# andrepxx/go-dsp-guitar

Hardware: AMD Instinct MI355X
Metric: Msamples/s through full chain incl. 64k-tap cab IR, 512ch@192kHz; %HBM roofline (higher is better)
Workload: dtype f64

## Files before the change

go-dsp-guitar_amd/csrc/api_ctx.cpp:

```cpp
#include "ctx.h"

static const int g_param_count[GDG_UNIT_COUNT] = { 6, 3, 3, 5, 4, 3, 7, 3, 7, 6, 4, 4, 2, 2, 3, 3, 1, 3, 1, 1, 1 };
static const int32_t g_param_default[GDG_UNIT_COUNT][GDG_MAX_PARAMS] = {
    { 100, 0, 0, 440, 100, 0 }, { -20, -40, 50 }, { 0, 300, 3000 }, { 1, -40, -10, 300, 6000 },
    { 1, -40, -10, 100 }, { 1, 30, -20 }, { 1, -20, -20, -20, -20, -20, -20 }, { 0, 0, 0 },
    { 1, 50, 0, 0, 100, 0, 0 }, { 0, 0, 100, 0, 1, 0 }, { 0, 0, 0, 0 }, { 0, -2, -5, -5 },
    { 100, 30 }, { 100, 10 }, { 100, 10, 45 }, { 100, 50, -10 }, { 100 }, { 200, -5, -5 }, { 50 }, { 14 }, { 0 },
};


const char *gdg_version(void) { return "gdg 0.1 gfx950 hip"; }

int gdg_device_count(void) {
    int n = 0;
    if (hipGetDeviceCount(&n) != hipSuccess) return 0;
    return n;
}


static bool parse_cpulist(const char *text, std::vector<int> &cpus) {
    cpus.clear();
    const char *p = text;
    while (*p && *p != '\n') {
        char *end = nullptr;
// ... 76 lines not shown
hipError_t pinned_alloc(gdg_ctx *ctx, void **p, size_t bytes) {
    const std::vector<int> *unused;
    const int node = numa_target(ctx, &unused);
    const bool bind = node >= 0 && node < 1024;
    if (bind) {
        unsigned long mask[16] = { 0 };
        mask[node / (8 * sizeof(unsigned long))] |= 1ul << (node % (8 * sizeof(unsigned long)));
        int old_mode = 0;
        unsigned long old_mask[16] = { 0 };
        const bool saved = syscall(SYS_get_mempolicy, &old_mode, old_mask, 1024ul + 1, nullptr, 0ul) == 0;
        const bool policy = saved && syscall(SYS_set_mempolicy, 1 , mask, 1024ul + 1) == 0;
        hipError_t e = hipHostMalloc(p, bytes, policy ? hipHostMallocNumaUser : hipHostMallocDefault);
        if (policy && syscall(SYS_set_mempolicy, old_mode, old_mode == 0 ? nullptr : old_mask, old_mode == 0 ? 0ul : 1024ul + 1) != 0)
            syscall(SYS_set_mempolicy, 0 , nullptr, 0ul);
        if (e == hipSuccess) return e;
        (void)hipGetLastError();
    }
    return hipHostMalloc(p, bytes, hipHostMallocDefault);
}

struct OptionDef {
    const char *key, *env;
    long long lo, hi;
    int knob;
    int gdg_ctx::*field;
    bool gdg_ctx::*flag;
    bool replans;
};
static const OptionDef g_options[] = {
    { "fir_fused", "GDG_FIR_FUSED", -1, 1, -1, &gdg_ctx::fir_fused, nullptr, true },
    { "fir_split_max_channels", "GDG_FIR_SPLIT_MAX", 0, 1 << 20, -1, &gdg_ctx::fir_split_max, nullptr, true },
    { "fir_split_max_channels_one_amp", "GDG_FIR_SPLIT_MAX_ONE_AMP", 0, 1 << 20, -1, &gdg_ctx::fir_split_max_single, nullptr, true },
    { "fir_chain_adjacent_amps", "GDG_FIR_CHAIN", 0, 1, -1, nullptr, &gdg_ctx::fir_chain, true },
    { "fir_premac", "GDG_FIR_PREMAC", 0, 1, -1, &gdg_ctx::fir_premac, nullptr, true },
    { "fir_premac_min_partitions", "GDG_FIR_PREMAC_MIN", 1, 1 << 24, -1, &gdg_ctx::fir_premac_min, nullptr, true },
    { "fir_premac_min_partitions_two_amps", "GDG_FIR_PREMAC_MIN_TWO", 1, 1 << 24, -1, &gdg_ctx::fir_premac_min_two, nullptr, true },
    { "stat_premac_launches_used", "GDG_STAT_PREMAC_USED", 0, 0x7fffffff, -1, &gdg_ctx::stat_premac_used, nullptr, false },
    { "stat_batch_device_kib", "GDG_STAT_BATCH_DEVICE_KIB", 0, 0x7fffffff, -1, &gdg_ctx::stat_batch_dev_kib, nullptr, false },
    { "stat_batch_upload_bytes", "GDG_STAT_BATCH_UPLOAD_BYTES", 0, 0x7fffffff, -1, &gdg_ctx::stat_batch_up_bytes, nullptr, false },
    { "stat_batch_resampled_samples", "GDG_STAT_BATCH_RESAMPLED", 0, 0x7fffffff, -1, &gdg_ctx::stat_batch_resampled, nullptr, false },
    { "fir_ahead_frames", "GDG_FIR_AHEAD", 0, 4, -1, &gdg_ctx::fir_ahead_frames, nullptr, true },
    { "fir_ahead_min_channels", "GDG_FIR_AHEAD_MIN", 1, 1 << 20, -1, &gdg_ctx::fir_ahead_min, nullptr, true },
    { "stat_fir_ahead_sums_used", "GDG_STAT_FIR_AHEAD_USED", 0, 0x7fffffff, -1, &gdg_ctx::stat_fir_ahead_used, nullptr, false },
    { "fir_premac_lds_bytes", "GDG_FIR_PREMAC_LDS", -1, 65536, -1, &gdg_ctx::fir_premac_lds, nullptr, true },
    { "share_ir_spectra", "GDG_SHARE_IR_SPECTRA", 0, 1, -1, nullptr, &gdg_ctx::share_spectra, false },
    { "fft_half_lds_mask", "GDG_FFT_HALF_LDS", 0, 63, GDG_KNOB_FFT_HALF_LDS, nullptr, nullptr, false },
    { "fir_forward_per_channel", "GDG_FWD_PER_CHANNEL", 0, 1, GDG_KNOB_FWD_PER_CHANNEL, nullptr, nullptr, false },
    { "fir_forward_wave_local", "GDG_WAVE_FFT", 0, 3, GDG_KNOB_WAVE_FFT, nullptr, nullptr, false },
    { "fir_mac_variant", "GDG_MAC_VARIANT", 0, 15, GDG_KNOB_MAC_VARIANT, nullptr, nullptr, false },
    { "seg_two_per_cu", "GDG_SEG_FAST", 0, 1, -1, nullptr, &gdg_ctx::seg_fast, true },
    { "seg_two_per_cu_min_channels", "GDG_SEG_FAST_MIN", 0, 1 << 20, -1, &gdg_ctx::seg_fast_min, nullptr, true },
    { "seg_wave_max_channels", "GDG_SEG_WAVE_MAX", 0, 1 << 20, -1, &gdg_ctx::seg_wave_max, nullptr, true },
    { "seg_wave_release_max_channels", "GDG_SEG_WAVE_RELEASE_MAX", 0, 1 << 20, -1, &gdg_ctx::seg_wave_release_max, nullptr, true },
    { "seg_tile_max_channels", "GDG_SEG_TILE_MAX", 0, 1 << 20, -1, &gdg_ctx::seg_tile_max, nullptr, true },
    { "seg_os_tiles_max_channels", "GDG_SEG_OS_TILES_MAX", 0, 1 << 20, -1, &gdg_ctx::seg_os_tiles_max, nullptr, true },
    { "seg_os_tiles_prefix", "GDG_SEG_OS_PREFIX", 0, 1, -1, nullptr, &gdg_ctx::seg_os_prefix, true },
    { "seg_reverb_ahead_max_channels", "GDG_SEG_REVERB_AHEAD_MAX", 0, 1 << 20, -1, &gdg_ctx::seg_reverb_ahead_max, nullptr, true },
    { "wave_spin_limit_ms", "GDG_WAVE_SPIN_LIMIT_MS", 1, 600000, -1, &gdg_ctx::wave_spin_ms, nullptr, false },
    { "debug_stall_unit", "GDG_DEBUG_STALL_UNIT", -1, 1 << 30, -1, &gdg_ctx::debug_stall_unit, nullptr, false },
    { "plan_patch", "GDG_PLAN_PATCH", 0, 1, -1, nullptr, &gdg_ctx::plan_patch, false },
    { "scan_tables_max", "GDG_SCAN_TABLES_MAX", 1, 1 << 20, -1, &gdg_ctx::scan_tables_max, nullptr, false },
    { "pcie_groups", "GDG_PCIE_GROUPS", 0, 16, -1, &gdg_ctx::pcie_groups_forced, nullptr, false },
    { "device_groups_default", "GDG_DEVICE_GROUPS", 0, 16, -1, &gdg_ctx::device_groups_env, nullptr, false },
    { "copy_threads", "GDG_COPY_THREADS", 1, 256, -1, &gdg_ctx::copy_threads, nullptr, false },
    { "numa", "GDG_NUMA", 0, 2, -1, &gdg_ctx::numa_mode, nullptr, false },
    { "tuner_parts", "GDG_TUNER_PARTS", 0, 24, GDG_KNOB_TUNER_PARTS, nullptr, nullptr, false },
// ... 515 lines not shown
```

go-dsp-guitar_amd/csrc/api_plan.cpp:

```cpp
#include "ctx.h"


static int ensure_hist(gdg_ctx *ctx, Unit &u, size_t len, long long key) {
    if (u.hist_key == key && u.hist_len == len) return GDG_OK;
    if (u.d_hist) { HIP_TRY(ctx, hipStreamSynchronize(ctx->stream)); ctx->arena.release(u.d_hist); u.d_hist = nullptr; }
    u.hist_len = len;
    u.hist_key = key;
    if (len > 0) {
        HIP_TRY(ctx, ctx->arena.alloc_zeroed((void **)&u.d_hist, len * sizeof(double), ctx->stream));
    }
    return GDG_OK;
}

static int zero_is(gdg_ctx *ctx, Unit &u, int first, int count) {
    HIP_TRY(ctx, hipMemsetAsync(u.d_is + first, 0, (size_t)count * sizeof(int), ctx->stream));
    return GDG_OK;
}

static double pow_u(double A, int e) {
    double r = 1.0, b = A;
    for (int k = 0; k < 10; k++) { if (e & (1 << k)) r *= b; b *= b; }
    return r;
}
static void lin_tab_host(bool maxop, double a, double keep, double *tab, int chk) {
    const double k2 = keep * keep, k4 = k2 * k2, A8 = k4 * k4, A = chk == 16 ? A8 * A8 : A8;
    for (int lane = 0; lane < 64; lane++) {
        tab[LT_PC_(chk) + lane] = pow_u(A, lane);
        if (lane < 16) tab[LT_PA_(chk) + lane] = pow_u(A, lane + 1);
        if (lane >= 32) tab[LT_PB_(chk) + lane - 32] = pow_u(A, lane - 31);
        if (lane < 10) tab[LT_ST_(chk) + lane] = pow_u(A, 1 << lane);
        if (lane < chk) tab[LT_W_(chk) + lane] = (maxop ? 1.0 : a) * pow_u(keep, chk - 1 - lane);
    }
}
// ... 540 lines not shown
    if (rc != GDG_OK) { u.fir_dirty = true; u.fir_live = false; return rc; }
    u.fir_P = P;
    u.fir_K = K;
    u.fir_R = R;
    u.fir_hop = hop;
    u.fir_dirty = false;
    u.fir_live = carry;
    return GDG_OK;
}

struct Op { bool is_fir; std::vector<int> handles; };
enum { K_SEG = 0, K_FIR = 1, K_OS2 = 2, K_OS4 = 3 };
struct PlanStep { int kind; std::vector<std::pair<int, Op>> ops; int unit_begin; };

static int wave_hand_off(const Unit &u, bool fast) {
    const int os = shaper_os_param(u.type);
    if (os >= 0 && u.params[os] == 0) return 0;
    const bool through = u.type == GDG_UNIT_COMPRESSOR || u.type == GDG_UNIT_TONESTACK || u.type == GDG_UNIT_CABINET || u.type == GDG_UNIT_CHORUS ||
                         u.type == GDG_UNIT_REVERB || (os >= 0 && !fast);
    return through ? 1 : 2;
}


static bool shapers_launch_alone(const gdg_ctx *ctx, int n_act, int frames) {
    return ctx->seg_os_tiles_max > 0 && n_act <= ctx->seg_os_tiles_max && frames == GDG_MAX_FRAMES;
}

#define GDG_TILE_WORKGROUP_BUDGET 224

struct Decisions {
    std::vector<char> fast;
    std::vector<char> made_ahead;
    std::vector<std::vector<int>> ahead;
};

static void decide_shapes(gdg_ctx *ctx, const std::vector<PlanStep> &plan, int n_act, int frames, uint32_t sample_rate, int G, int n_units, Decisions &dec) {
    std::vector<StepDesc> &steps = ctx->steps;
    const size_t S = steps.size();
    const bool batch = frames == GDG_MAX_FRAMES;
    dec.fast.assign(S, 0);
    dec.made_ahead.assign((size_t)n_units, 0);
    dec.ahead.assign(S, std::vector<int>());
    int fir_steps = 0;
    for (auto &st : steps) fir_steps += st.is_fir ? 1 : 0;

    const int split_max = fir_steps >= 2 ? ctx->fir_split_max : std::min(ctx->fir_split_max, ctx->fir_split_max_single);
    auto fused = [&](int n) { return ctx->fir_fused < 0 ? n > split_max : ctx->fir_fused != 0; };
    const long premac_min = fir_steps >= 2 ? std::min(ctx->fir_premac_min, ctx->fir_premac_min_two) : ctx->fir_premac_min;
    int premac_steps = 0;
    const int ahead_T = ctx->fir_ahead_frames >= 2 ? ctx->fir_ahead_frames : 0;
    int ahead_steps = 0;
    for (size_t i = 0; i < S; i++) {
        StepDesc &st = steps[i];
        if (!st.is_fir) continue;
        long partitions = 0;
        bool every_k2 = true;
        for (auto &e : plan[i].ops) {
            const int K = ctx->units[(size_t)e.second.handles[0]].fir_K;
            partitions += K;
            every_k2 = every_k2 && K >= 2;
        }
        const bool premac = ctx->fir_premac != 0 && !fused(st.n) && G == 1 && batch && every_k2 && partitions >= premac_min;
        premac_steps += premac ? 1 : 0;
        bool ahead_pays = true;
        for (auto &e : plan[i].ops) {
            const long K = ctx->units[(size_t)e.second.handles[0]].fir_K;
// ... 67 lines not shown
    }
    const bool tiles = n_act <= ctx->seg_tile_max && G == 1 && batch && !(premac_steps >= 2 && n_act > ctx->seg_reverb_ahead_max);
    for (size_t i = 0; i < S; i++) {
        StepDesc &st = steps[i];
        if (st.is_fir) continue;
        if (st.os_factor) {
            st.window = Shape::OS_TILES;
            st.runs[0].frame = st.os_prefix_step >= 0 ? Shape::OS_TILES_PREFIX : Shape::OS_TILES;
            for (auto &r : st.runs) r.frame = st.runs[0].frame;
            continue;
        }
        const bool fast = dec.fast[i] != 0;
        bool release = false;
        int unit = plan[i].unit_begin;
        for (auto &e : plan[i].ops)
            for (int h : e.second.handles) release = release || wave_hand_off(ctx->units[(size_t)h], fast) == 2;
        const int wave_max = release ? std::min(ctx->seg_wave_max, ctx->seg_wave_release_max) : ctx->seg_wave_max;
        const bool wave = n_act <= wave_max && st.wave_tickets >= 0;
        st.window = fast ? (wave ? Shape::SEGF_WAVE : Shape::SEGF_WALK) : (wave ? Shape::WAVE : Shape::WALK);
        bool tile = tiles && !fast && st.wave_tickets >= 0 && 2 * st.n + (int)dec.ahead[i].size() <= GDG_TILE_WORKGROUP_BUDGET;
        for (auto &e : plan[i].ops) {
            int xids = 0;
            for (int h : e.second.handles) {
                const Unit &tu = ctx->units[(size_t)h];
                const int os = shaper_os_param(tu.type);
                if (!gdg_segt_supported(tu.type) || (os >= 0 && tu.params[os] != 0) || (gdg_segt_supported(tu.type) == 2 && !dec.made_ahead[(size_t)unit])) tile = false;
                xids += gdg_segt_exchanges(tu.type);
                unit++;
            }
            if (xids > 32 || e.second.handles.size() > 16 || e.second.handles.empty()) tile = false;
        }
        const Shape frame = skip[i] ? Shape::SKIP : fast ? Shape::SEGF : tile ? Shape::SEGT : dec.ahead[i].empty() ? Shape::GENERAL : Shape::GENERAL_AHEAD;
        for (auto &r : st.runs) r.frame = frame;
    }
}

int build_plan(gdg_ctx *ctx, const std::vector<int> &active, const double *d_in, double *d_out, int frames, uint32_t sample_rate,
                      int stride, int stride_out, bool rows_by_channel, int G, const std::vector<size_t> &bounds) {
    const int nch = ctx->nch;
    int ptrace = 0;
    { const char *e = getenv("GDG_PLAN_TRACE"); ptrace = e ? atoi(e) : 0; }
    ctx->plan_trace = ptrace;
    auto pnow = []() { return std::chrono::duration<double, std::milli>(std::chrono::steady_clock::now().time_since_epoch()).count(); };
    double t_fir = 0.0, t_unit = 0.0;
    const double t_plan0 = pnow();
    join_groups(ctx);
    join_premac(ctx, false);
    drop_fir_ahead(ctx);
    {
        long limit = ctx->scan_tables_max;
        if (limit < 1) limit = 1;
        if ((long)ctx->scan_tabs.size() > limit) {
            HIP_TRY(ctx, hipStreamSynchronize(ctx->stream));
            for (auto &kv : ctx->scan_tabs) ctx->arena.release(kv.second);
            ctx->scan_tabs.clear();
        }
    }
    const int n_act = (int)active.size();
    std::vector<int> group_of((size_t)nch, 0);
    for (int g = 0; g < G; g++)
        for (size_t i = bounds[(size_t)g]; i < bounds[(size_t)g + 1]; i++) group_of[(size_t)active[i]] = g;
    ctx->plan_groups = G;
    std::map<int, std::vector<std::pair<int, Op>>> by_slot;
    std::vector<int> n_ops((size_t)nch, 0);
    std::vector<int> row_of((size_t)nch, -1);
    for (size_t i = 0; i < active.size(); i++) row_of[(size_t)active[i]] = rows_by_channel ? active[i] : (int)i;
// ... 48 lines not shown
        st.is_fir = ps.kind == K_FIR;
        st.os_factor = ps.kind == K_OS2 ? 2 : ps.kind == K_OS4 ? 4 : 0;
        st.n = (int)ps.ops.size();
        st.offset = 0;
        st.runs.assign((size_t)G, StepDesc::Run());
        for (int pos = 0; pos < st.n; pos++) {
            auto &r = st.runs[(size_t)group_of[(size_t)ps.ops[(size_t)pos].first]];
            if (r.n == 0) r.first = pos;
            r.n++;
        }
        if (!st.is_fir) {
            for (auto &e : ps.ops) n_units += (int)e.second.handles.size();
            if (seg_steps < GDG_WAVE_STEPS && G <= GDG_WAVE_GROUPS) st.wave_tickets = GDG_WAVE_GROUPS * seg_steps++;
        }
        ctx->steps.push_back(st);
        plan.push_back(std::move(ps));
    }
    for (auto &ps : plan) {
        if (ps.kind != K_FIR) continue;
        for (auto &e : ps.ops) {
            const double tq = pnow();
            int rc = prepare_fir(ctx, ctx->units[(size_t)e.second.handles[0]], frames, sample_rate);
            t_fir += pnow() - tq;
            if (rc != GDG_OK) return rc;
        }
    }
    Decisions dec;
    decide_shapes(ctx, plan, n_act, frames, sample_rate, G, n_units, dec);
    size_t wave_next = (size_t)GDG_WAVE_STEPS * GDG_WAVE_GROUPS;
    std::vector<gdg_seg_unit> seg_units;
    std::vector<std::vector<gdg_seg_chan>> seg_descs;
    std::vector<std::vector<gdg_fir_chan>> fir_descs;
    std::vector<int> done((size_t)nch, 0);
    std::vector<const double *> cur((size_t)nch);
    for (int c : active) cur[(size_t)c] = d_in + (size_t)row_of[(size_t)c] * stride;
    ctx->plan_unit_slot.assign(ctx->units.size(), -1);
    ctx->patch_units.clear();
    ctx->plan_unit_fast.assign(ctx->units.size(), 0);
    ctx->plan_unit_fast_ok.assign(ctx->units.size(), 0);
    bool acc_synced = false;
    for (size_t i = 0; i < plan.size(); i++) {
        StepDesc &st = ctx->steps[i];
        const bool step_fast = dec.fast[i] != 0;
        std::vector<gdg_seg_chan> sd;
        std::vector<gdg_fir_chan> fd;
        for (auto &entry : plan[i].ops) {
            int c = entry.first;
            const Op &op = entry.second;
            bool last = (done[(size_t)c] + 1 == n_ops[(size_t)c]);
            double *dst;
            if (last) dst = d_out + (size_t)row_of[(size_t)c] * stride_out;
            else dst = ((done[(size_t)c] & 1) ? ctx->d_w1 : ctx->d_w0) + (size_t)c * ctx->w_stride;
            if (st.is_fir) {
                Unit &u = ctx->units[(size_t)op.handles[0]];
                const size_t need = (size_t)st.fir_ahead_T * (size_t)u.fir_P * sizeof(double2);
                if (u.acc_bytes < need || (need == 0 && u.d_acc)) {
                    if (!acc_synced) { HIP_TRY(ctx, hipStreamSynchronize(ctx->stream)); acc_synced = true; }
                    ctx->arena.release(u.d_acc);
                    u.d_acc = nullptr;
                    u.acc_bytes = 0;
                    if (need) { HIP_TRY(ctx, ctx->arena.alloc((void **)&u.d_acc, need)); u.acc_bytes = need; }
                }
                gdg_fir_chan f;
                memset(&f, 0, sizeof(f));
                f.src = cur[(size_t)c]; f.dst = dst; f.prev = u.d_prev; f.fdl = u.d_fdl; f.H = u.H->d_H; f.Y = u.d_Y;
                f.pos = u.d_pos; f.K = u.fir_K; f.R = u.fir_R; f.hop = frames;
                f.acc = st.fir_ahead_T > 0 ? u.d_acc : nullptr;
                f.flags = (done[(size_t)c] == 0 ? GDG_SRC_IS_INPUT : 0) | (last ? GDG_DST_IS_OUTPUT : 0) |
                          (st.chain_next ? GDG_DST_UNUSED : 0);
                fd.push_back(f);
                u.fir_live = true;
            } else {
                gdg_seg_chan s;
                memset(&s, 0, sizeof(s));
                s.src = cur[(size_t)c]; s.dst = dst;
                s.flags = (done[(size_t)c] == 0 ? GDG_SRC_IS_INPUT : 0) | (last ? GDG_DST_IS_OUTPUT : 0);
                s.scratch = ctx->d_scratch + (size_t)c * ctx->max_frames;
                s.unit_begin = (int)seg_units.size();
                s.unit_count = (int)op.handles.size();
                s.wave = ctx->d_wave + wave_next;
                wave_next += 8 * op.handles.size();
                {
                    unsigned mask = 0;
                    for (size_t ui = 0; ui < op.handles.size(); ui++) {
                        const Unit &wu = ctx->units[(size_t)op.handles[ui]];
                        const int hand_off = wave_hand_off(wu, step_fast);
                        if (hand_off == 0) continue;
                        if (ui < 15) mask |= 1u << ui;
                        if (ui < 15 && (wu.type == GDG_UNIT_COMPRESSOR || wu.type == GDG_UNIT_TONESTACK || wu.type == GDG_UNIT_CABINET))
                            mask |= 1u << (16 + ui);
                        if (hand_off == 2) mask |= 1u << 31;
                    }
                    s.wave_mask = (int)mask;
                }
                for (int h : op.handles) {
                    gdg_seg_unit du;
                    const double tq = pnow();
                    int rc = prepare_unit(ctx, ctx->units[(size_t)h], frames, sample_rate, du, step_fast ? GDG_CHK_FAST : GDG_CHK);
                    t_unit += pnow() - tq;
                    if (rc != GDG_OK) return rc;
                    if (du.type == GDG_UNIT_REVERB && du.jp[4] != std::max(std::max(du.jp[0], du.jp[1]), std::max(du.jp[2], du.jp[3])) + GDG_MAX_FRAMES)
                        return fail(ctx, GDG_ERR_INVALID, "reverb delay line of %d cells, expected the longest tap + %d", du.jp[4], GDG_MAX_FRAMES);
                    if (du.type == GDG_UNIT_REVERB) du.ip[7] = dec.made_ahead[seg_units.size()];
                    ctx->plan_unit_slot[(size_t)h] = (int)seg_units.size();
                    ctx->plan_unit_fast[(size_t)h] = step_fast ? 1 : 0;
                    ctx->plan_unit_fast_ok[(size_t)h] = segf_unit_ok(ctx->units[(size_t)h], frames, sample_rate) ? 1 : 0;
                    seg_units.push_back(du);
                }
                sd.push_back(s);
            }
            cur[(size_t)c] = dst;
            done[(size_t)c]++;
        }
        if (st.os_factor) { st.os_flags = (int)wave_next; wave_next += sd.size(); st.os_arrive = (int)wave_next; wave_next += sd.size(); }
        if (st.is_fir) {
            std::vector<const void *> hp;
            for (auto &f : fd) hp.push_back(f.H);
            std::sort(hp.begin(), hp.end());
            st.shared_spectra = std::adjacent_find(hp.begin(), hp.end()) != hp.end();
        }
        seg_descs.push_back(sd);
        fir_descs.push_back(fd);
    }
    {
        const double tq = pnow();
        int rc = flush_ir(ctx);
        if (ptrace) fprintf(stderr, "[plan] prepare_fir %.1f ms, prepare_unit %.1f ms, flush_ir %.1f ms, so far %.1f ms\n", t_fir, t_unit, pnow() - tq, pnow() - t_plan0);
        if (rc != GDG_OK) return rc;
    }
    ctx->blob.clear();
    auto append = [&](const void *p, size_t bytes) {
        size_t off = (ctx->blob.size() + 255) & ~(size_t)255;
        ctx->blob.resize(off + bytes);
        if (bytes) memcpy(ctx->blob.data() + off, p, bytes);
        return off;
    };
    for (size_t i = 0; i < ctx->steps.size(); i++) {
        if (ctx->steps[i].is_fir) ctx->steps[i].offset = append(fir_descs[i].data(), fir_descs[i].size() * sizeof(gdg_fir_chan));
        else ctx->steps[i].offset = append(seg_descs[i].data(), seg_descs[i].size() * sizeof(gdg_seg_chan));
    }
    ctx->units_offset = append(seg_units.data(), seg_units.size() * sizeof(gdg_seg_unit));
// ... 38 lines not shown
```

go-dsp-guitar_amd/csrc/ctx.h:

```cpp
#ifndef GDG_CTX_H
#define GDG_CTX_H

#include "../../include/gdg.h"
#include "gdg_internal.h"
#include "aa_taps.h"
#include "go_consts.h"
#include "notes.h"

#include <math.h>
#include <stdarg.h>
#include <stdio.h>
#include <string.h>

#include <unistd.h>
#include <pthread.h>
#include <sched.h>
#include <sys/syscall.h>

#include <algorithm>
#include <atomic>
#include <chrono>
#include <condition_variable>
#include <functional>
#include <mutex>
// ... 167 lines not shown
    bool premac_valid = false;
    bool premac_outstanding = false;
    int seg_reverb_ahead_max = 72;
    int wave_spin_ms = 1000;
    int debug_stall_unit = -1;
    int wave_epoch = 0;
    int *d_wave = nullptr;
    size_t d_wave_cap = 0;
    std::vector<int> patch_units;
    bool plan_patch = true;
    int plan_trace = 0;
    std::vector<unsigned char> blob;
    unsigned char *d_blob = nullptr;
    size_t d_blob_cap = 0;
    size_t units_offset = 0;
    double *d_w0 = nullptr, *d_w1 = nullptr, *d_scratch = nullptr;
    int window = 1;
    size_t w_stride = 0;
    double *d_stage_in = nullptr, *d_stage_out = nullptr;
    double *h_stage_in = nullptr, *h_stage_out = nullptr;
    int stage_out_stride = 0;
    int stage_out_frames = 0;
    int *d_error = nullptr;
    DevArena arena;
    std::map<std::vector<double>, double *> scan_tabs;
    std::vector<void *> user_allocs;
    std::map<int, std::pair<double2 *, double2 *>> fir_tables;
    std::multimap<uint64_t, std::weak_ptr<SharedSpectra>> spectra;
    std::vector<std::shared_ptr<SharedSpectra>> pending_ir;
    bool share_spectra = true;
    int fir_fused = -1;
    int fir_split_max = 192;
    int fir_split_max_single = 112;
    bool fir_chain = true;
    double *d_os = nullptr;
    gdg_os_tables os;
    unsigned profiling = 0;
    int prof_every = 1;
    unsigned long long prof_calls = 0;
    bool prof_now = true;
    bool prof_attach = true;
    std::vector<ProfEvent> prof;
    std::vector<hipEvent_t> event_pool;
    double *d_tuner_ring = nullptr;
    int tuner_wp = 0;
    uint32_t tuner_sr = 0;
    double *d_note_freqs = nullptr;
    gdg_tuner_out *d_tuner_out = nullptr, *h_tuner_out = nullptr;
    double2 *d_tuner_work = nullptr, *d_tuner_twn = nullptr, *d_tuner_twm = nullptr;
    int tuner_part_cap = 0;
    unsigned tuner_seq = 0;
    int tuner_poll = 1;
    double2 *d_tuner_part = nullptr;
    std::vector<double> sp_az, sp_dist, sp_level;
    uint32_t sp_hist_sr = 96000;
    double *d_sp_hist = nullptr;
    int sp_hist_len = 0, sp_hist_cur = 0;
    gdg_spat_chan *d_sp_chan = nullptr;
    double *d_sp_out = nullptr;
    bool sp_dirty = true;
    void *d_io[2] = { nullptr, nullptr };
    size_t io_cap[2] = { 0, 0 };
    gdg_meter_rec *d_meter = nullptr;
    int n_meter = 0;
    PinnedHalves h_batch;
    hipStream_t batch_stream = nullptr;
// ... 304 lines not shown
```

go-dsp-guitar_amd/csrc/fir.hip:

```cpp
#include "gdg_internal.h"
#include <hip/hip_ext.h>
#include <math.h>
#include <stdlib.h>
#include <type_traits>
#include <vector>

typedef double2 cplx;

__device__ __forceinline__ cplx cadd(cplx a, cplx b) { return make_double2(a.x + b.x, a.y + b.y); }
__device__ __forceinline__ cplx csub(cplx a, cplx b) { return make_double2(a.x - b.x, a.y - b.y); }
#pragma clang fp contract(off)
__device__ __forceinline__ cplx cmul(cplx a, cplx b) {
    return make_double2(__builtin_fma(a.x, b.x, -(a.y * b.y)), __builtin_fma(a.x, b.y, a.y * b.x));
}

typedef double v2d __attribute__((ext_vector_type(2)));
#define GDG_GLOBAL __attribute__((address_space(1)))
__device__ __forceinline__ cplx gload(const cplx *p) {
    v2d v = *reinterpret_cast<const GDG_GLOBAL v2d *>((const GDG_GLOBAL void *)p);
    return make_double2(v.x, v.y);
}
__device__ __forceinline__ void gstore(cplx *p, cplx c) {
    v2d v = { c.x, c.y };
    *reinterpret_cast<GDG_GLOBAL v2d *>((GDG_GLOBAL void *)p) = v;
// ... 202 lines not shown
    meet();
    pass_store1<LOGN, LR, LNS, 1>(v, s, tid);
    meet();
    pass_load1<LOGN, LR1, 1>(v, s, tid);
}

template <int LOGN, bool IRJOB>
__global__ void __launch_bounds__(FftCfg<LOGN>::T)
fir_fwd_kernel(const gdg_fir_chan *__restrict__ chans, const gdg_fir_irjob *__restrict__ jobs, double scale, gdg_shift shift,
               const cplx *__restrict__ tw, const cplx *__restrict__ tw2) {
    constexpr int N = FftCfg<LOGN>::N, T = FftCfg<LOGN>::T;
    __shared__ double sre[FftCfg<LOGN>::LDS];
    __shared__ double sim[FftCfg<LOGN>::LDS];
    const int tid = threadIdx.x;
    const double *a, *bsrc;
    double *prev_out = nullptr;
    cplx *out;
    int hop = N;
    if constexpr (IRJOB) {
        gdg_fir_irjob jb = jobs[blockIdx.x];
        a = jb.a;
        bsrc = jb.b;
        out = jb.out;
        if (jb.hop > 0) hop = jb.hop;
        else bsrc = nullptr;
    } else {
        gdg_fir_chan ch = chans[blockIdx.x];
        int pos = *ch.pos;
        a = ch.prev + (size_t)((pos + 1) & 1) * N;
        prev_out = ch.prev + (size_t)(pos & 1) * N;
        bsrc = (ch.flags & GDG_SRC_IS_INPUT) ? ch.src + shift.in : ch.src;
        out = ch.fdl + (size_t)(pos % ch.R) * N;
        hop = ch.hop;
    }

    constexpr int LR0 = sched_lr(LOGN, 0), R0 = 1 << LR0, B0 = 16 / R0;
    cplx v[16];
#pragma unroll
    for (int b = 0; b < B0; b++) {
        int j = tid + T * b;
#pragma unroll
        for (int t = 0; t < R0; t++) {
            int e = j + t * (N / R0);
            cplx val;
            if ((!IRJOB && hop != N) || (IRJOB && bsrc != nullptr)) {
                double r2[2];
#pragma unroll
                for (int h = 0; h < 2; h++) {
                    const int i = 2 * e + h;
                    double x = 0.0;
                    if (i < hop) x = gload1(a + i);
                    else if (i < 2 * hop) { x = gload1(bsrc + (i - hop)); if constexpr (!IRJOB) gstore1(prev_out + (i - hop), x); }
                    r2[h] = x;
                }
                val = make_double2(r2[0], r2[1]);
            } else if (e < N / 2) {
                val = gload(reinterpret_cast<const cplx *>(a + 2 * e));
            } else {
                if constexpr (IRJOB) val = make_double2(0.0, 0.0);
                else {
                    val = gload(reinterpret_cast<const cplx *>(bsrc + 2 * (e - N / 2)));
                    gstore(reinterpret_cast<cplx *>(prev_out + 2 * (e - N / 2)), val);
                }
            }
            v[b * R0 + t] = val;
        }
    }
    pass_compute<LOGN, LR0, 0, false>(v, tw, tid);
    pass_store<LOGN, LR0, 0>(v, sre, sim, tid);
    __syncthreads();
    run_lds_passes<LOGN, 1, sched_npass(LOGN), false>(v, sre, sim, tw, tid);

    constexpr int ITER = (N / 2) / T;
#pragma unroll
    for (int i = 0; i < ITER; i++) {
        int k = tid + T * i;
        if (k == 0) {
            double zx = sre[0], zy = sim[0];
            gstore(out, make_double2((zx + zy) * scale, (zx - zy) * scale));
            double hx = sre[GDG_PAD(N / 2)], hy = sim[GDG_PAD(N / 2)];
            gstore(out + N / 2, make_double2(hx * scale, -hy * scale));
        } else {
            int n = N - k;
            cplx zk = make_double2(sre[GDG_PAD(k)], sim[GDG_PAD(k)]);
            cplx zn = make_double2(sre[GDG_PAD(n)], sim[GDG_PAD(n)]);
            cplx A = make_double2(zk.x + zn.x, zk.y - zn.y);
            cplx Bv = make_double2(zk.x - zn.x, zk.y + zn.y);
            cplx cw = cmul(tw2[k], Bv);
            double hs = 0.5 * scale;
            gstore(out + k, make_double2((A.x + cw.y) * hs, (A.y - cw.x) * hs));
            gstore(out + n, make_double2((A.x - cw.y) * hs, (-A.y - cw.x) * hs));
        }
    }
}

// ... 9 lines not shown
    pass_compute<L, 4, 0, INV, 8>(v, tw, lane);
    pass_store<L, 4, 0>(v, rre, rim, lane);
    __builtin_amdgcn_wave_barrier();
    pass_load<L, 3>(v, rre, rim, lane);
    __builtin_amdgcn_wave_barrier();
    pass_compute<L, 3, 4, INV, 8>(v, tw, lane);
    pass_store<L, 3, 4>(v, rre, rim, lane);
    __builtin_amdgcn_wave_barrier();
    pass_load<L, 3>(v, rre, rim, lane);
    __builtin_amdgcn_wave_barrier();
    pass_compute<L, 3, 7, INV, 8>(v, tw, lane);
}

__device__ __forceinline__ void twiddle_powers8(cplx (&u)[8], cplx w) {
    cplx w2 = cmul(w, w), w4 = cmul(w2, w2), w3 = cmul(w2, w), w5 = cmul(w4, w), w6 = cmul(w4, w2), w7 = cmul(w4, w3);
    u[1] = cmul(u[1], w); u[2] = cmul(u[2], w2); u[3] = cmul(u[3], w3); u[4] = cmul(u[4], w4);
    u[5] = cmul(u[5], w5); u[6] = cmul(u[6], w6); u[7] = cmul(u[7], w7);
}

template <int TB>
__global__ void __launch_bounds__(512)
fir_fwd13w_kernel(const gdg_fir_chan *__restrict__ chans, int W, gdg_shift shift, const cplx *__restrict__ tw, const cplx *__restrict__ tw2) {
    constexpr int N = 8192, T = 512;
    __shared__ double sre[GDG_W_LDS];
    __shared__ double sim[GDG_W_LDS];
    const int tid = threadIdx.x, wave = tid >> 6, lane = tid & 63;
    const int jw = TB ? (int)(blockIdx.x % (unsigned)W) : 0;
    gdg_fir_chan ch = chans[TB ? blockIdx.x / (unsigned)W : blockIdx.x];
    if (ch.flags & GDG_SRC_IS_INPUT) ch.src += shift.in;
    const int pos = *ch.pos;
    const double *a = ch.prev + (size_t)((pos + 1) & 1) * N;
    if (TB && jw > 0) a = ch.src + (size_t)jw * N - N;
    double *prev_out = ch.prev + (size_t)(pos & 1) * N;
    const double *bsrc = ch.src + (size_t)jw * N;
    cplx *out = ch.fdl + (size_t)((pos + jw) % ch.R) * N;

    cplx ua[2][8], wa[2];
#pragma unroll
    for (int b = 0; b < 2; b++) {
        const int n1 = tid + T * b;
        wa[b] = tw[n1];
#pragma unroll
        for (int n2 = 0; n2 < 8; n2++) {
            const int e = n1 + 1024 * n2;
            ua[b][n2] = (n2 < 4) ? gload(reinterpret_cast<const cplx *>(a + 2 * e)) : gload(reinterpret_cast<const cplx *>(bsrc + 2 * (e - N / 2)));
        }
    }
#pragma unroll
    for (int b = 0; b < 2; b++) {
        const int n1 = tid + T * b;
        if constexpr (!TB) {
#pragma unroll
            for (int n2 = 4; n2 < 8; n2++) gstore(reinterpret_cast<cplx *>(prev_out + 2 * (n1 + 1024 * n2 - N / 2)), ua[b][n2]);
        }
        Dft<8, false>::run(ua[b]);
        twiddle_powers8(ua[b], wa[b]);
#pragma unroll
        for (int k2 = 0; k2 < 8; k2++) { sre[k2 * GDG_W_RL + GDG_PAD(n1)] = ua[b][k2].x; sim[k2 * GDG_W_RL + GDG_PAD(n1)] = ua[b][k2].y; }
    }
    __syncthreads();
    {
        double *rre = sre + wave * GDG_W_RL, *rim = sim + wave * GDG_W_RL;
        cplx v[16];
        wave_fft1024<false>(v, rre, rim, tw, lane);
        __builtin_amdgcn_wave_barrier();
#pragma unroll
        for (int b = 0; b < 2; b++)
#pragma unroll
            for (int t = 0; t < 8; t++) {
                const int k1 = (lane + 64 * b) + 128 * t;
                rre[GDG_PAD(k1)] = v[b * 8 + t].x;
                rim[GDG_PAD(k1)] = v[b * 8 + t].y;
            }
    }
    __syncthreads();
    auto Z = [&](int k) { return make_double2(sre[(k & 7) * GDG_W_RL + GDG_PAD(k >> 3)], sim[(k & 7) * GDG_W_RL + GDG_PAD(k >> 3)]); };
#pragma unroll
    for (int i = 0; i < 8; i++) {
        const int k = tid + T * i;
        if (k == 0) {
            cplx z0 = Z(0), zh = Z(N / 2);
            gstore(out, make_double2(z0.x + z0.y, z0.x - z0.y));
            gstore(out + N / 2, make_double2(zh.x, -zh.y));
        } else {
            const int n = N - k;
            cplx zk = Z(k), zn = Z(n);
            cplx A = make_double2(zk.x + zn.x, zk.y - zn.y);
            cplx Bv = make_double2(zk.x - zn.x, zk.y + zn.y);
            cplx cw = cmul(tw2[k], Bv);
            gstore(out + k, make_double2((A.x + cw.y) * 0.5, (A.y - cw.x) * 0.5));
            gstore(out + n, make_double2((A.x - cw.y) * 0.5, (-A.y - cw.x) * 0.5));
        }
    }
}

template <int TB>
__global__ void __launch_bounds__(512, 4)
fir_fwd13wh_kernel(const gdg_fir_chan *__restrict__ chans, int W, gdg_shift shift, const cplx *__restrict__ tw, const cplx *__restrict__ tw2, int by_xcd) {
    constexpr int N = 8192, T = 512;
    __shared__ double s[GDG_W_LDS];
    const int tid = threadIdx.x, wave = tid >> 6, lane = tid & 63;
    unsigned cw = TB ? blockIdx.x / (unsigned)W : blockIdx.x, jw = TB ? blockIdx.x % (unsigned)W : 0u;
    if (TB && by_xcd) {
        const unsigned x = blockIdx.x & 7u, q = blockIdx.x >> 3;
        cw = x + 8u * (q / (unsigned)W);
        jw = q % (unsigned)W;
    }
    gdg_fir_chan ch = chans[cw];
    if (ch.flags & GDG_SRC_IS_INPUT) ch.src += shift.in;
    const int pos = *ch.pos;
    const double *a = ch.prev + (size_t)((pos + 1) & 1) * N;
    if (TB && jw > 0) a = ch.src + (size_t)jw * N - N;
    double *prev_out = ch.prev + (size_t)(pos & 1) * N;
    const double *bsrc = ch.src + (size_t)jw * N;
    cplx *out = ch.fdl + (size_t)((pos + jw) % ch.R) * N;

    cplx ua[2][8], wa[2];
#pragma unroll
    for (int b = 0; b < 2; b++) {
        const int n1 = tid + T * b;
        wa[b] = tw[n1];
#pragma unroll
        for (int n2 = 0; n2 < 8; n2++) {
            const int e = n1 + 1024 * n2;
            ua[b][n2] = (n2 < 4) ? gload(reinterpret_cast<const cplx *>(a + 2 * e)) : gload(reinterpret_cast<const cplx *>(bsrc + 2 * (e - N / 2)));
        }
    }
#pragma unroll
    for (int b = 0; b < 2; b++) {
        const int n1 = tid + T * b;
        if constexpr (!TB) {
#pragma unroll
            for (int n2 = 4; n2 < 8; n2++) gstore(reinterpret_cast<cplx *>(prev_out + 2 * (n1 + 1024 * n2 - N / 2)), ua[b][n2]);
        }
        Dft<8, false>::run(ua[b]);
        twiddle_powers8(ua[b], wa[b]);
#pragma unroll
        for (int k2 = 0; k2 < 8; k2++) s[k2 * GDG_W_RL + GDG_PAD(n1)] = ua[b][k2].x;
    }
    double *rs = s + wave * GDG_W_RL;
    cplx v[16];
    __syncthreads();
    pass_load1<10, 4, 0>(v, rs, lane);
    __syncthreads();
#pragma unroll
    for (int b = 0; b < 2; b++)
#pragma unroll
        for (int k2 = 0; k2 < 8; k2++) s[k2 * GDG_W_RL + GDG_PAD(tid + T * b)] = ua[b][k2].y;
    __syncthreads();
    pass_load1<10, 4, 1>(v, rs, lane);
    pass_compute<10, 4, 0, false, 8>(v, tw, lane);
    exchange1<10, 0, true>(v, rs, lane);
    pass_compute<10, 3, 4, false, 8>(v, tw, lane);
    exchange1<10, 1, true>(v, rs, lane);
    pass_compute<10, 3, 7, false, 8>(v, tw, lane);
    auto Zs = [&](int k) { return s[(k & 7) * GDG_W_RL + GDG_PAD(k >> 3)]; };
    double zkx[8], znx[8];
    __builtin_amdgcn_wave_barrier();
    int ln = lane;
    asm volatile("" : "+v"(ln));
    double *rn = rs + GDG_PAD(ln);
#pragma unroll
    for (int b = 0; b < 2; b++)
#pragma unroll
        for (int t = 0; t < 8; t++) rn[GDG_PAD(64 * b + 128 * t)] = v[b * 8 + t].x;
    __syncthreads();
// ... 1145 lines not shown
```

go-dsp-guitar_amd/csrc/gdg_internal.h:

```cpp
#ifndef GDG_INTERNAL_H
#define GDG_INTERNAL_H

#include <hip/hip_runtime.h>
#include <stdint.h>

#define GDG_MAX_FRAMES 8192
#define GDG_MIN_FIR_FRAMES 64

#define GDG_SRC_IS_INPUT 1
#define GDG_DST_IS_OUTPUT 2
#define GDG_DST_UNUSED 4
struct gdg_shift { long long in, out; };

struct gdg_fir_chan {
    const double *src;
    double *dst;
    double *prev;
    double2 *fdl;
    const double2 *H;
    double2 *Y;
    int *pos;
    double2 *acc;
    int K;
    int R;
    int flags;
    int hop;
};

struct gdg_fir_irjob {
    const double *a;
    double2 *out;
    const double *b;
    int hop;
    int pad;
};

struct gdg_fir_rawjob {
    const double2 *Y;
    double *first, *second;
    int hop, pad;
};

enum { GDG_KNOB_FFT_HALF_LDS = 0, GDG_KNOB_FWD_PER_CHANNEL, GDG_KNOB_WAVE_FFT, GDG_KNOB_MAC_VARIANT, GDG_KNOB_TUNER_PARTS, GDG_KNOB_COUNT };
int gdg_knob_get(int which);
// ... 42 lines not shown
#define LT_ST_(c) (c)
#define LT_PA_(c) ((c) + 10)
#define LT_PB_(c) ((c) + 26)
#define LT_PC_(c) ((c) + 58)
#define LT_SIZE_(c) ((c) + 122)
#define L2_W_(c) 0
#define L2_ST_(c) (2 * (c))
#define L2_PA_(c) (2 * (c) + 30)
#define L2_PB_(c) (2 * (c) + 78)
#define L2_PC_(c) (2 * (c) + 174)
#define L2_SIZE_(c) (2 * (c) + 366)
#define LT_W LT_W_(GDG_CHK)
#define LT_ST LT_ST_(GDG_CHK)
#define LT_PA LT_PA_(GDG_CHK)
#define LT_PB LT_PB_(GDG_CHK)
#define LT_PC LT_PC_(GDG_CHK)
#define LT_SIZE LT_SIZE_(GDG_CHK)
#define L2_W L2_W_(GDG_CHK)
#define L2_ST L2_ST_(GDG_CHK)
#define L2_PA L2_PA_(GDG_CHK)
#define L2_PB L2_PB_(GDG_CHK)
#define L2_PC L2_PC_(GDG_CHK)
#define L2_SIZE L2_SIZE_(GDG_CHK)

struct gdg_seg_chan {
    const double *src;
    double *dst;
    double *scratch;
    int unit_begin;
    int unit_count;
    int flags;
    int wave_mask;
    int *wave;
};

struct gdg_os_tables {
    const double *taps2;
    const double *taps4;
    const double *lanczos2;
    const double *lanczos4;
    const double *tapsP2;
    const double *tapsP4;
};
#define GDG_OS_TAPS(F) ((F) == 2 ? 77 : 155)
#define GDG_OS_BACK(F) ((GDG_OS_TAPS(F) - 1 + (F) - 1) / (F))
#define GDG_OS_R(F) ((F) == 2 ? 4 : 2)
#define GDG_OS_NC 48
#define GDG_OS_PADLO(F) (GDG_OS_NC - 1 - GDG_OS_BACK(F))
#define GDG_OS_NE(F) (GDG_OS_NC + GDG_OS_R(F) - 1 + 1)

hipError_t gdg_launch_seg(const gdg_seg_chan *d_chans, int n_chans, const gdg_seg_unit *d_units, int frames, int n_frames, gdg_shift shift,
                          gdg_os_tables os, int *d_error, hipStream_t s, int *d_wave_ticket = nullptr, int epoch = 0, int ahead = 0,
                          const int *d_ahead_list = nullptr, int n_ahead = 0);
hipError_t gdg_launch_segf(const gdg_seg_chan *d_chans, int n_chans, const gdg_seg_unit *d_units, int frames, int n_frames, gdg_shift shift,
                           gdg_os_tables os, int *d_error, hipStream_t s, int *d_wave_ticket = nullptr, int epoch = 0, int ahead = 0,
                           const int *d_ahead_list = nullptr, int n_ahead = 0);
int gdg_segf_supported(int unit_type);
hipError_t gdg_launch_segt(const gdg_seg_chan *d_chans, int n_chans, const gdg_seg_unit *d_units, gdg_shift shift, gdg_os_tables os, int *d_error,
                           hipStream_t s, int *d_ticket, int epoch, unsigned long long *d_xch, const int *d_ahead_list, int n_ahead);
int gdg_segt_supported(int unit_type);
int gdg_segt_exchanges(int unit_type);
size_t gdg_segt_xch_words(void);
hipError_t gdg_launch_os_tiles(int factor, const gdg_seg_chan *d_chans, int n_chans, const gdg_seg_unit *d_units, int frames, int n_frames,
                               gdg_shift shift, gdg_os_tables os, int *d_flags, int epoch, int *d_error, hipStream_t s,
                               const gdg_seg_chan *d_pre_chans = nullptr, int *d_arrive = nullptr);
hipError_t gdg_launch_os_debug(int factor, const double *d_in, int n, double *d_hist, double *d_up, double *d_down, gdg_os_tables os, hipStream_t s);
// ... 82 lines not shown
```

go-dsp-guitar_amd/csrc/seg.hip:

```cpp
#ifdef SEG_FAST
#define GDG_CHK 16
#endif
#include "gdg_internal.h"
#include "go_consts.h"
#include "../../include/gdg.h"
#include <math.h>
#include <stdlib.h>

#ifdef SEG_FAST
#define SEG_T 512
#define SEG_MIN_WAVES_PER_EU 4
#define SEG_SCR 1600
#define seg_kernel segf_kernel
#define gdg_launch_seg gdg_launch_segf
#define gdg_seg_supported gdg_segf_supported
#elif defined(SEG_TILE)
#define SEG_T 512
#define SEG_MIN_WAVES_PER_EU 2
#define SEG_SCR 3328
#define SEG_TILES 2
#else
#define SEG_T 1024
#define SEG_MIN_WAVES_PER_EU 4
#define SEG_SCR 3328
// ... 2698 lines not shown
        for (int i = tid; i < N / 2; i += SEG_T) { seg_v2d v = { fin[LX(2 * i)], fin[LX(2 * i + 1)] }; d2[i] = v; }
    } else {
        for (int i = tid; i < N; i += SEG_T) as_global(dst)[i] = fin[LX(i)];
    }
}
#ifdef SEG_FAST
#define SEG_KERNEL_ATTR __attribute__((amdgpu_num_vgpr(60)))
#else
#define SEG_KERNEL_ATTR
#endif
#ifdef SEG_TILE
#define GDG_TILE_XCH_WORDS (GDG_TILE_XIDS * 16 * 2 * 2)
__global__ void __launch_bounds__(SEG_T, SEG_MIN_WAVES_PER_EU)
segt_kernel(const gdg_seg_chan *__restrict__ chans, const gdg_seg_unit *__restrict__ units, gdg_shift shift, gdg_os_tables os, int *d_error,
            int n_chans, int *ticket, int epoch, unsigned long long *xch, const int *__restrict__ ahead_list) {
    const int tid = seg_tid();
    if ((int)blockIdx.x >= SEG_TILES * n_chans) {
        const WaveGate none = {};
        reverb_general<REVERB_AHEAD>(units + ahead_list[blockIdx.x - SEG_TILES * n_chans], 0, GDG_MAX_FRAMES, false, none);
        return;
    }
    int *s_ticket = reinterpret_cast<int *>(s_tmp + SEG_STASH + 32) + 16;
    if (tid == 0) {
        const int t = atomicAdd(ticket, 1);
        if (t == SEG_TILES * n_chans - 1) __hip_atomic_store(as_global(ticket), 0, __ATOMIC_RELAXED, __HIP_MEMORY_SCOPE_AGENT);
        *s_ticket = t;
    }
    __syncthreads();
    const int t = __builtin_amdgcn_readfirstlane(*s_ticket);
    const int tile = t / n_chans, block = t - tile * n_chans;
    gdg_seg_chan ch = chans[block];
    if (ch.flags & GDG_SRC_IS_INPUT) ch.src += shift.in;
    if (ch.flags & GDG_DST_IS_OUTPUT) ch.dst += shift.out;
    if (tid == 0) { s_tc.xch = xch + (size_t)block * GDG_TILE_XCH_WORDS; s_tc.d_error = d_error; s_tc.tile = tile; s_tc.epoch = epoch; s_tc.xid = 0; }
    int my_type = 0;
    if (tid < ch.unit_count && tid < 16) my_type = *(const GDG_GLOBAL int *)&units[ch.unit_begin + tid].type;
    seg_frame<false>(ch.src + (size_t)tile * SEG_N, ch.dst + (size_t)tile * SEG_N, units, ch.unit_begin, ch.unit_count, SEG_N, os, d_error, my_type);
}

int gdg_segt_supported(int unit_type) {
    switch (unit_type) {
    case GDG_UNIT_COMPRESSOR: case GDG_UNIT_OVERDRIVE: case GDG_UNIT_DISTORTION: case GDG_UNIT_EXCESS: case GDG_UNIT_TONESTACK:
    case GDG_UNIT_CABINET: case GDG_UNIT_CHORUS:
        return 1;
    case GDG_UNIT_REVERB:
        return 2;
    default:
        return 0;
    }
}
int gdg_segt_exchanges(int unit_type) {
    return unit_type == GDG_UNIT_COMPRESSOR ? 1 : unit_type == GDG_UNIT_TONESTACK ? 4 : unit_type == GDG_UNIT_CABINET ? 7 :
           (unit_type == GDG_UNIT_CHORUS || unit_type == GDG_UNIT_REVERB) ? 1 : 0;
}
size_t gdg_segt_xch_words(void) { return GDG_TILE_XCH_WORDS; }

hipError_t gdg_launch_segt(const gdg_seg_chan *d_chans, int n_chans, const gdg_seg_unit *d_units, gdg_shift shift, gdg_os_tables os, int *d_error,
                           hipStream_t s, int *d_ticket, int epoch, unsigned long long *d_xch, const int *d_ahead_list, int n_ahead) {
    if (n_chans <= 0) return hipSuccess;
    if (!d_ahead_list) n_ahead = 0;
    hipLaunchKernelGGL(segt_kernel, dim3(SEG_TILES * n_chans + n_ahead), dim3(SEG_T), 0, s, d_chans, d_units, shift, os, d_error, n_chans, d_ticket, epoch, d_xch, d_ahead_list);
    return hipGetLastError();
}
#else
template <int MODE>
__global__ void __launch_bounds__(SEG_T, SEG_MIN_WAVES_PER_EU) SEG_KERNEL_ATTR
seg_kernel(const gdg_seg_chan *__restrict__ chans, const gdg_seg_unit *__restrict__ units, int N, int n_frames, gdg_shift shift,
           gdg_os_tables os, int *d_error, int n_chans, int *ticket, int epoch, int ahead, const int *__restrict__ ahead_list) {
    constexpr bool MULTI = MODE == 1;
    int block = blockIdx.x, wf0 = 0;
#ifndef SEG_FAST
    if (MODE == 0 && block >= n_chans) {
        const WaveGate none = {};
        reverb_general<REVERB_AHEAD>(units + ahead_list[block - n_chans], 0, GDG_MAX_FRAMES, false, none);
        return;
    }
#endif
    if (MODE == 2) {
        int *s_ticket = reinterpret_cast<int *>(s_tmp + SEG_STASH + 32) + 16;
        if (threadIdx.x == 0) {
            const int t = atomicAdd(ticket, 1);
            if (t == n_chans * n_frames - 1) __hip_atomic_store(as_global(ticket), 0, __ATOMIC_RELAXED, __HIP_MEMORY_SCOPE_AGENT);
            *s_ticket = t;
        }
        __syncthreads();
        const int t = __builtin_amdgcn_readfirstlane(*s_ticket);
        wf0 = t / n_chans;
        block = t - wf0 * n_chans;
    }
    gdg_seg_chan ch = chans[block];
    if (ch.flags & GDG_SRC_IS_INPUT) ch.src += shift.in;
    if (ch.flags & GDG_DST_IS_OUTPUT) ch.dst += shift.out;
    const int tid = seg_tid();
    int my_type = 0;
    if (tid < ch.unit_count && tid < 16) my_type = *(const GDG_GLOBAL int *)&units[ch.unit_begin + tid].type;
    if (MODE == 2) {
        seg_frame<true>(ch.src + (size_t)wf0 * N, ch.dst + (size_t)wf0 * N, units, ch.unit_begin, ch.unit_count, N, os, d_error, my_type,
                        ch.wave, wf0, wf0 + 1 < n_frames ? wf0 + 1 : 0, (unsigned)ch.wave_mask, epoch, 0, ahead );
        return;
    }
    for (int wf = 0; wf < (MULTI ? n_frames : 1); wf++, ch.src += N, ch.dst += N) {
        seg_frame<false>(ch.src, ch.dst, units, ch.unit_begin, ch.unit_count, N, os, d_error, my_type, nullptr, 0, 0, 0, 0, MODE == 0 ? ahead : 0);
        if (MULTI && wf + 1 < n_frames) { __threadfence_block(); __syncthreads(); }
    }
}

int gdg_seg_supported(int unit_type) {
#ifdef SEG_FAST
    switch (unit_type) {
    case GDG_UNIT_COMPRESSOR: case GDG_UNIT_OVERDRIVE: case GDG_UNIT_DISTORTION: case GDG_UNIT_EXCESS: case GDG_UNIT_TONESTACK:
    case GDG_UNIT_CABINET: case GDG_UNIT_CHORUS: case GDG_UNIT_RINGMODULATOR: case GDG_UNIT_TREMOLO: case GDG_UNIT_SIGNALGENERATOR:
    case GDG_UNIT_REVERB:
        return 1;
    default:
        return 0;
    }
#endif
    switch (unit_type) {
    case GDG_UNIT_COMPRESSOR: case GDG_UNIT_OVERDRIVE: case GDG_UNIT_DISTORTION: case GDG_UNIT_EXCESS:
    case GDG_UNIT_TONESTACK: case GDG_UNIT_CABINET: case GDG_UNIT_CHORUS: case GDG_UNIT_FLANGER:
    case GDG_UNIT_PHASER: case GDG_UNIT_DELAY: case GDG_UNIT_RINGMODULATOR: case GDG_UNIT_TREMOLO:
    case GDG_UNIT_SIGNALGENERATOR: case GDG_UNIT_REVERB: case GDG_UNIT_FUZZ: case GDG_UNIT_AUTOYOY:
    case GDG_UNIT_AUTOWAH: case GDG_UNIT_BANDPASS: case GDG_UNIT_OCTAVER: case GDG_UNIT_NOISEGATE:
        return 1;
    default:
// ... 22 lines not shown
```

Baseline: 9872.

## Write segment output directly into FIR history slot to skip copy

When a segment kernel feeds a partitioned FIR whose partition equals the frame size, the segment kernel now writes its output straight into the FIR's double-buffered history slot (chosen from the FIR position counter). The FIR forward kernels then read that slot as their input and skip storing the input copy into history. This removes one full write and re-read of each channel's frame between stages, at the cost of coupling the segment kernel to the FIR's slot state. The option is on by default. There is a risk of mismatch if the slot position is read before the FIR's position has advanced, and the MODE 2 and multi-frame paths do not redirect their output.

```diff
diff --git a/go-dsp-guitar_amd/csrc/api_ctx.cpp b/go-dsp-guitar_amd/csrc/api_ctx.cpp
--- a/go-dsp-guitar_amd/csrc/api_ctx.cpp
+++ b/go-dsp-guitar_amd/csrc/api_ctx.cpp
@@ -132,6 +132,8 @@
     { "fir_split_max_channels", "GDG_FIR_SPLIT_MAX", 0, 1 << 20, -1, &gdg_ctx::fir_split_max, nullptr, true },
     { "fir_split_max_channels_one_amp", "GDG_FIR_SPLIT_MAX_ONE_AMP", 0, 1 << 20, -1, &gdg_ctx::fir_split_max_single, nullptr, true },
     { "fir_chain_adjacent_amps", "GDG_FIR_CHAIN", 0, 1, -1, nullptr, &gdg_ctx::fir_chain, true },
+    { "fir_history_slots", "GDG_FIR_HISTORY_SLOTS", 0, 1, -1, &gdg_ctx::fir_history_slots, nullptr, true },
+    { "stat_fir_history_slot_channels", "GDG_STAT_FIR_SLOT_CHANNELS", 0, 0x7fffffff, -1, &gdg_ctx::stat_fir_slot_channels, nullptr, false },
     { "fir_premac", "GDG_FIR_PREMAC", 0, 1, -1, &gdg_ctx::fir_premac, nullptr, true },
     { "fir_premac_min_partitions", "GDG_FIR_PREMAC_MIN", 1, 1 << 24, -1, &gdg_ctx::fir_premac_min, nullptr, true },
     { "fir_premac_min_partitions_two_amps", "GDG_FIR_PREMAC_MIN_TWO", 1, 1 << 24, -1, &gdg_ctx::fir_premac_min_two, nullptr, true },
diff --git a/go-dsp-guitar_amd/csrc/api_plan.cpp b/go-dsp-guitar_amd/csrc/api_plan.cpp
--- a/go-dsp-guitar_amd/csrc/api_plan.cpp
+++ b/go-dsp-guitar_amd/csrc/api_plan.cpp
@@ -1,4 +1,5 @@
 #include "ctx.h"
+#include "fir_slots.h"
 
 
 static int ensure_hist(gdg_ctx *ctx, Unit &u, size_t len, long long key) {
@@ -605,6 +606,7 @@
     std::vector<char> fast;
     std::vector<char> made_ahead;
     std::vector<std::vector<int>> ahead;
+    std::vector<std::vector<int>> slot_from;
 };
 
 static void decide_shapes(gdg_ctx *ctx, const std::vector<PlanStep> &plan, int n_act, int frames, uint32_t sample_rate, int G, int n_units, Decisions &dec) {
@@ -738,6 +740,29 @@
         }
         const Shape frame = skip[i] ? Shape::SKIP : fast ? Shape::SEGF : tile ? Shape::SEGT : dec.ahead[i].empty() ? Shape::GENERAL : Shape::GENERAL_AHEAD;
         for (auto &r : st.runs) r.frame = frame;
+    }
+
+    dec.slot_from.assign(S, std::vector<int>());
+    {
+        std::map<int, std::pair<int, int>> last;
+        for (size_t i = 0; i < S; i++) {
+            const StepDesc &st = steps[i];
+            int producer = GDG_PRODUCER_FIR;
+            if (!st.is_fir) {
+                const Shape f = st.runs[0].frame;
+                producer = (f == Shape::GENERAL || f == Shape::GENERAL_AHEAD || f == Shape::SEGF || f == Shape::SEGT) ? GDG_PRODUCER_SEGMENT : GDG_PRODUCER_OS_TILES;
+            } else dec.slot_from[i].assign(plan[i].ops.size(), -1);
+            for (size_t k = 0; k < plan[i].ops.size(); k++) {
+                const int c = plan[i].ops[k].first;
+                if (st.is_fir) {
+                    auto it = last.find(c);
+                    const int from = it == last.end() ? GDG_PRODUCER_INPUT : it->second.second;
+                    const Unit &u = ctx->units[(size_t)plan[i].ops[k].second.handles[0]];
+                    if (gdg_fir_slot_direct(ctx->fir_history_slots, from, frames, u.fir_P)) dec.slot_from[i][k] = it->second.first;
+                }
+                last[c] = { (int)i, producer };
+            }
+        }
     }
 }
 
@@ -852,6 +877,8 @@
     std::vector<std::vector<gdg_seg_chan>> seg_descs;
     std::vector<std::vector<gdg_fir_chan>> fir_descs;
     std::vector<int> done((size_t)nch, 0);
+    std::vector<int> seg_desc_of((size_t)nch, -1);
+    ctx->stat_fir_slot_channels = 0;
     std::vector<const double *> cur((size_t)nch);
     for (int c : active) cur[(size_t)c] = d_in + (size_t)row_of[(size_t)c] * stride;
     ctx->plan_unit_slot.assign(ctx->units.size(), -1);
@@ -888,6 +915,14 @@
                 f.acc = st.fir_ahead_T > 0 ? u.d_acc : nullptr;
                 f.flags = (done[(size_t)c] == 0 ? GDG_SRC_IS_INPUT : 0) | (last ? GDG_DST_IS_OUTPUT : 0) |
                           (st.chain_next ? GDG_DST_UNUSED : 0);
+                const int from = dec.slot_from[i][fd.size()];
+                if (from >= 0) {
+                    gdg_seg_chan &producer = seg_descs[(size_t)from][(size_t)seg_desc_of[(size_t)c]];
+                    producer.slot = u.d_prev;
+                    producer.slot_pos = u.d_pos;
+                    f.flags |= GDG_SRC_IS_SLOT;
+                    stat_add(ctx->stat_fir_slot_channels);
+                }
                 fd.push_back(f);
                 u.fir_live = true;
             } else {
@@ -927,6 +962,7 @@
                     ctx->plan_unit_fast_ok[(size_t)h] = segf_unit_ok(ctx->units[(size_t)h], frames, sample_rate) ? 1 : 0;
                     seg_units.push_back(du);
                 }
+                seg_desc_of[(size_t)c] = (int)sd.size();
                 sd.push_back(s);
             }
             cur[(size_t)c] = dst;
diff --git a/go-dsp-guitar_amd/csrc/ctx.h b/go-dsp-guitar_amd/csrc/ctx.h
--- a/go-dsp-guitar_amd/csrc/ctx.h
+++ b/go-dsp-guitar_amd/csrc/ctx.h
@@ -223,6 +223,8 @@
     int fir_fused = -1;
     int fir_split_max = 192;
     int fir_split_max_single = 112;
+    int fir_history_slots = 1;
+    int stat_fir_slot_channels = 0;
     bool fir_chain = true;
     double *d_os = nullptr;
     gdg_os_tables os;
diff --git a/go-dsp-guitar_amd/csrc/fir.hip b/go-dsp-guitar_amd/csrc/fir.hip
--- a/go-dsp-guitar_amd/csrc/fir.hip
+++ b/go-dsp-guitar_amd/csrc/fir.hip
@@ -258,6 +258,7 @@
         bsrc = (ch.flags & GDG_SRC_IS_INPUT) ? ch.src + shift.in : ch.src;
         out = ch.fdl + (size_t)(pos % ch.R) * N;
         hop = ch.hop;
+        if (ch.flags & GDG_SRC_IS_SLOT) { bsrc = prev_out; prev_out = nullptr; }
     }
 
     constexpr int LR0 = sched_lr(LOGN, 0), R0 = 1 << LR0, B0 = 16 / R0;
@@ -276,7 +277,7 @@
                     const int i = 2 * e + h;
                     double x = 0.0;
                     if (i < hop) x = gload1(a + i);
-                    else if (i < 2 * hop) { x = gload1(bsrc + (i - hop)); if constexpr (!IRJOB) gstore1(prev_out + (i - hop), x); }
+                    else if (i < 2 * hop) { x = gload1(bsrc + (i - hop)); if constexpr (!IRJOB) if (prev_out) gstore1(prev_out + (i - hop), x); }
                     r2[h] = x;
                 }
                 val = make_double2(r2[0], r2[1]);
@@ -286,7 +287,7 @@
                 if constexpr (IRJOB) val = make_double2(0.0, 0.0);
                 else {
                     val = gload(reinterpret_cast<const cplx *>(bsrc + 2 * (e - N / 2)));
-                    gstore(reinterpret_cast<cplx *>(prev_out + 2 * (e - N / 2)), val);
+                    if (prev_out) gstore(reinterpret_cast<cplx *>(prev_out + 2 * (e - N / 2)), val);
                 }
             }
             v[b * R0 + t] = val;
@@ -362,7 +363,8 @@
     const double *a = ch.prev + (size_t)((pos + 1) & 1) * N;
     if (TB && jw > 0) a = ch.src + (size_t)jw * N - N;
     double *prev_out = ch.prev + (size_t)(pos & 1) * N;
-    const double *bsrc = ch.src + (size_t)jw * N;
+    const bool kept = !TB && (ch.flags & GDG_SRC_IS_SLOT);
+    const double *bsrc = kept ? prev_out : ch.src + (size_t)jw * N;
     cplx *out = ch.fdl + (size_t)((pos + jw) % ch.R) * N;
 
     cplx ua[2][8], wa[2];
@@ -380,8 +382,10 @@
     for (int b = 0; b < 2; b++) {
         const int n1 = tid + T * b;
         if constexpr (!TB) {
-#pragma unroll
-            for (int n2 = 4; n2 < 8; n2++) gstore(reinterpret_cast<cplx *>(prev_out + 2 * (n1 + 1024 * n2 - N / 2)), ua[b][n2]);
+            if (!kept) {
+#pragma unroll
+                for (int n2 = 4; n2 < 8; n2++) gstore(reinterpret_cast<cplx *>(prev_out + 2 * (n1 + 1024 * n2 - N / 2)), ua[b][n2]);
+            }
         }
         Dft<8, false>::run(ua[b]);
         twiddle_powers8(ua[b], wa[b]);
@@ -442,7 +446,8 @@
     const double *a = ch.prev + (size_t)((pos + 1) & 1) * N;
     if (TB && jw > 0) a = ch.src + (size_t)jw * N - N;
     double *prev_out = ch.prev + (size_t)(pos & 1) * N;
-    const double *bsrc = ch.src + (size_t)jw * N;
+    const bool kept = !TB && (ch.flags & GDG_SRC_IS_SLOT);
+    const double *bsrc = kept ? prev_out : ch.src + (size_t)jw * N;
     cplx *out = ch.fdl + (size_t)((pos + jw) % ch.R) * N;
 
     cplx ua[2][8], wa[2];
@@ -460,8 +465,10 @@
     for (int b = 0; b < 2; b++) {
         const int n1 = tid + T * b;
         if constexpr (!TB) {
-#pragma unroll
-            for (int n2 = 4; n2 < 8; n2++) gstore(reinterpret_cast<cplx *>(prev_out + 2 * (n1 + 1024 * n2 - N / 2)), ua[b][n2]);
+            if (!kept) {
+#pragma unroll
+                for (int n2 = 4; n2 < 8; n2++) gstore(reinterpret_cast<cplx *>(prev_out + 2 * (n1 + 1024 * n2 - N / 2)), ua[b][n2]);
+            }
         }
         Dft<8, false>::run(ua[b]);
         twiddle_powers8(ua[b], wa[b]);
diff --git a/go-dsp-guitar_amd/csrc/fir_slots.h b/go-dsp-guitar_amd/csrc/fir_slots.h
--- /dev/null
+++ b/go-dsp-guitar_amd/csrc/fir_slots.h
@@ -0,0 +1,20 @@
+#ifndef GDG_FIR_SLOTS_H
+#define GDG_FIR_SLOTS_H
+
+static inline int gdg_fir_slot_current(int pos) { return pos & 1; }
+static inline int gdg_fir_slot_previous(int pos) { return (pos + 1) & 1; }
+static inline int gdg_fir_pos_advance(int pos, int n, int R) { return (int)(((long long)pos + n) % (2ll * R)); }
+static inline int gdg_fir_slot_history(int pos) { return gdg_fir_slot_previous(pos); }
+static inline long long gdg_fir_slot_offset(int slot, int P) { return (long long)slot * P; }
+
+enum gdg_slot_producer {
+    GDG_PRODUCER_INPUT = 0,
+    GDG_PRODUCER_FIR,
+    GDG_PRODUCER_OS_TILES,
+    GDG_PRODUCER_SEGMENT
+};
+static inline int gdg_fir_slot_direct(int option_on, int producer, int frames, int P) {
+    return option_on != 0 && producer == GDG_PRODUCER_SEGMENT && frames == P;
+}
+
+#endif
diff --git a/go-dsp-guitar_amd/csrc/gdg_internal.h b/go-dsp-guitar_amd/csrc/gdg_internal.h
--- a/go-dsp-guitar_amd/csrc/gdg_internal.h
+++ b/go-dsp-guitar_amd/csrc/gdg_internal.h
@@ -10,6 +10,7 @@
 #define GDG_SRC_IS_INPUT 1
 #define GDG_DST_IS_OUTPUT 2
 #define GDG_DST_UNUSED 4
+#define GDG_SRC_IS_SLOT 8
 struct gdg_shift { long long in, out; };
 
 struct gdg_fir_chan {
@@ -118,6 +119,8 @@
     int flags;
     int wave_mask;
     int *wave;
+    double *slot;
+    const int *slot_pos;
 };
 
 struct gdg_os_tables {
diff --git a/go-dsp-guitar_amd/csrc/seg.hip b/go-dsp-guitar_amd/csrc/seg.hip
--- a/go-dsp-guitar_amd/csrc/seg.hip
+++ b/go-dsp-guitar_amd/csrc/seg.hip
@@ -2754,6 +2754,7 @@
     gdg_seg_chan ch = chans[block];
     if (ch.flags & GDG_SRC_IS_INPUT) ch.src += shift.in;
     if (ch.flags & GDG_DST_IS_OUTPUT) ch.dst += shift.out;
+    if (ch.slot_pos) ch.dst = ch.slot + (size_t)(__builtin_amdgcn_readfirstlane(*(const GDG_GLOBAL int *)ch.slot_pos) & 1) * GDG_MAX_FRAMES;
     if (tid == 0) { s_tc.xch = xch + (size_t)block * GDG_TILE_XCH_WORDS; s_tc.d_error = d_error; s_tc.tile = tile; s_tc.epoch = epoch; s_tc.xid = 0; }
     int my_type = 0;
     if (tid < ch.unit_count && tid < 16) my_type = *(const GDG_GLOBAL int *)&units[ch.unit_begin + tid].type;
@@ -2813,6 +2814,7 @@
     gdg_seg_chan ch = chans[block];
     if (ch.flags & GDG_SRC_IS_INPUT) ch.src += shift.in;
     if (ch.flags & GDG_DST_IS_OUTPUT) ch.dst += shift.out;
+    if (MODE == 0 && ch.slot_pos) ch.dst = ch.slot + (size_t)(__builtin_amdgcn_readfirstlane(*(const GDG_GLOBAL int *)ch.slot_pos) & 1) * N;
     const int tid = seg_tid();
     int my_type = 0;
     if (tid < ch.unit_count && tid < 16) my_type = *(const GDG_GLOBAL int *)&units[ch.unit_begin + tid].type;
```

Result: no change. 9927 (median of 2 runs) (+0.6%).
